# OpenGene/repaq

Hardware: AMD Instinct MI355X
Metric: raw FASTQ MB/s encode+decode (higher is better)
Workload: dtype u8; 1 GPU; configs[2]: synthetic NovaSeq PE150 two files (-i/-I), 2 x 4.01 GB FASTQ (fqgen profile 1, 11200000 pairs, seed 3, N 20 ppm), -k 1000, encode + decode; chunks_per_gpu=3360, parity=unchecked (checked with --full)

## Files before the change

### repaq_amd/csrc/enc/chunk_flags_overlap.h

```cpp
#pragma once
struct Layout {
    uint32_t off_readlens, off_n1lens, off_n2lens, off_stlens, off_lanes, off_tiles, off_x, off_y, off_n1, off_n2, off_st, off_seq, off_qual, off_ov, off_npos;
    uint32_t total, msize, seq_size, qual_size, npos_size, n1_size, n2_size, st_size, x_size, y_size, n_reads, flags;
};
__device__ __forceinline__ uint32_t name2_len_of(const Text& T, const ReadTab& R, uint32_t g) { return line_len(T, g, 0) - R.name2_off[g]; }

#define CF_ALL 0x3FFu
__global__ void k_chunk_flags_a(Text T, ReadTab R, ChunkTab C, const DevHeader* __restrict__ D, int is_pe, uint32_t* __restrict__ cbits, uint32_t* __restrict__ cfail) {
    __shared__ uint8_t s_names[4 * 65 * NAME_STRIDE];
    const uint32_t c = blockIdx.y, f = C.first[c], e = C.first[c + 1];
    const int l = lane_id(), w = wave_id(); const uint32_t wpb = blockDim.x >> 6;
    uint8_t* rows = s_names + (size_t)w * 65 * NAME_STRIDE;
    const bool can0 = is_pe && D->support_interleaved; const uint32_t dpos = D->name2_diff_pos, dch = D->name2_diff_char;
    const uint32_t nl0 = line_len(T, f, 0); const uint8_t* nm0g = line_ptr(T, f, 0);
    const uint32_t n1l0 = R.name1_len[f], n2o0 = R.name2_off[f], n2l0 = nl0 - n2o0, len0 = R.len[f], stl0 = line_len(T, f, 2);
    const uint8_t* st0 = line_ptr(T, f, 2); const uint8_t lane0 = R.lane[f]; const uint16_t tile0 = R.tile[f];
    { const uint32_t take = nl0 < NAME_CAP ? nl0 : NAME_CAP; for (uint32_t i = (uint32_t)l; i < take; i += 64) rows[64 * NAME_STRIDE + i] = nm0g[i]; }
    const uint8_t* nm0 = nl0 <= NAME_CAP ? rows + 64 * NAME_STRIDE : nm0g;
    uint32_t bits = CF_ALL, fail = 0xFFFFFFFFu;
    for (uint32_t gb = f + (blockIdx.x * wpb + (uint32_t)w) * 64u; gb < e; gb += gridDim.x * wpb * 64u) {
        const uint32_t g = gb + (uint32_t)l; const bool v = g < e;
        uint32_t nb = 0, nl = 0, stb = 0, stl = 0; int s = 0;
        if (v) { uint32_t r; read_loc(T, g, s, r); const uint32_t* p = t_lo(T, s) + 4 * (size_t)r; nb = p[0]; nl = p[1] - 1 - nb; stb = p[2]; stl = p[3] - 1 - stb; }
        wave_lds_sync();
// ... 81 lines not shown
}
#define OV2_CROW_OF(capb) ((capb) / 4u + 4u)
#define OV2_NROW_OF(capb) ((capb) == 256u ? 36u : (capb) / 8u + 8u)
#define OV2_FILTER 8
__device__ __forceinline__ uint32_t bfe_u32(uint32_t v, uint32_t off, uint32_t wid) { return (v >> off) & ((1u << wid) - 1u); }
static __device__ __noinline__ uint4 ld16_edge(const uint8_t* __restrict__ base, long long off, uint64_t n) {
    uint32_t w[4] = { 0, 0, 0, 0 };
    for (int b = 0; b < 16; b++) { const long long a = off + b; if (a >= 0 && (uint64_t)a < n) w[b >> 2] |= (uint32_t)base[a] << (8 * (b & 3)); }
    return make_uint4(w[0], w[1], w[2], w[3]);
}
__device__ __forceinline__ void ov2_pack_r1(uint32_t w, uint32_t& code, uint32_t& nbits, uint32_t& bad) {
    const uint32_t idx = (w >> 1) & 0x03030303u;
    const uint32_t ok = eq_bytes_full(__builtin_amdgcn_perm(0u, 0x47544341u, idx), w);
    code = ((__builtin_amdgcn_perm(0u, 0x00020301u, idx) & ok) * 0x01041040u) >> 24;
    nbits = 0; bad = 0;
    if (ok != 0xFFFFFFFFu) { const uint32_t isn = eq_bytes_full(w, 0x4E4E4E4Eu); nbits = ((isn & 0x01010101u) * 0x01020408u) >> 24; bad = ~ok & ~isn; }
}
__device__ __forceinline__ void ov2_pack_rc(uint32_t w, uint32_t& code, uint32_t& nbits) {
    const uint32_t u = w & 0xDFDFDFDFu, idx = (u >> 1) & 0x03030303u;
    const uint32_t ok = eq_bytes_full(__builtin_amdgcn_perm(0u, 0x47544341u, idx), u);
    code = ((__builtin_amdgcn_perm(0u, 0x03010002u, idx) & ok) * 0x01041040u) >> 24;
    nbits = ((~ok & 0x01010101u) * 0x01020408u) >> 24;
}
struct OvLoose { const uint32_t* pq; const uint32_t* lpk; const uint16_t* lnb; const uint8_t* rflag; };
template <bool LOOSE, uint32_t CAPB = 256u> __global__ void __launch_bounds__(256) k_overlap(Text T, OvLoose Z, int16_t* __restrict__ ovraw, uint32_t n_pairs) {
    constexpr uint32_t OV2_CAP = CAPB, OV2_CROW = OV2_CROW_OF(CAPB), OV2_NROW = OV2_NROW_OF(CAPB), OV2_WAVE_BYTES = 128u * (OV2_CROW + OV2_NROW); constexpr int OV2_ND = (int)(CAPB / 16u);
    static_assert((OV2_CROW / 4u) % 2u == 1u && (OV2_NROW / 4u) % 2u == 1u && OV2_WAVE_BYTES % 16u == 0u, "row geometry");
    __shared__ uint32_t s_rows[4 * (OV2_WAVE_BYTES / 4) + 4]; __shared__ uint32_t s_bad[4][2];
    const int l = lane_id(), w = wave_id();
    uint8_t* const c1 = (uint8_t*)(s_rows + (size_t)w * (OV2_WAVE_BYTES / 4)); uint8_t* const c2 = c1 + 64u * OV2_CROW;
    uint8_t* const n1 = c2 + 64u * OV2_CROW; uint8_t* const n2 = n1 + 64u * OV2_NROW;
    for (uint32_t p0 = (blockIdx.x * 4u + (uint32_t)w) * 64u; p0 < n_pairs; p0 += gridDim.x * 256u) {
        const uint32_t p = p0 + (uint32_t)l; int len1 = -1, len2 = 0; uint32_t q1 = 0, q2 = 0; int s1 = 0, s2 = 0; uint32_t ld1 = 0, ld2 = 0;
        if (p < n_pairs) {
            const uint32_t g = 2u * p;
            if (LOOSE) { const uint32_t a = Z.pq[g], b = Z.pq[g + 1], c_ = Z.pq[g + 2]; len1 = (int)(b - a); len2 = (int)(c_ - b); ld1 = (a >> 4) + g;
                    ld2 = (b >> 4) + g + 1u; }
            else { uint32_t r; read_loc(T, g, s1, r); const uint32_t* pa = t_lo(T, s1) + 4 * (size_t)r; q1 = pa[1]; len1 = (int)(pa[2] - 1u - q1);
                              read_loc(T, g + 1, s2, r); const uint32_t* pb = t_lo(T, s2) + 4 * (size_t)r; q2 = pb[1]; len2 = (int)(pb[2] - 1u - q2); }
        }
        const bool slow = len1 >= 0 && ((uint32_t)len1 > OV2_CAP || (uint32_t)len2 > OV2_CAP), fast = len1 >= 0 && !slow;
        const int mx = wave_max(fast ? (len1 > len2 ? len1 : len2) : 0);
        if (l < 2) s_bad[w][l] = 0;
        wave_lds_sync();
        { uint4* z = (uint4*)c1; for (uint32_t i = (uint32_t)l; i < OV2_WAVE_BYTES / 16u; i += 64u) z[i] = make_uint4(0, 0, 0, 0); }
        wave_lds_sync();
        if (LOOSE) {
            const uint32_t nd_ = ((uint32_t)mx + 15u) >> 4;
            uint32_t* const r1w = (uint32_t*)(c1 + (uint32_t)l * OV2_CROW); uint32_t* const r2w = (uint32_t*)(c2 + (uint32_t)l * OV2_CROW);
            uint16_t* const m1w = (uint16_t*)(n1 + (uint32_t)l * OV2_NROW); uint16_t* const m2w = (uint16_t*)(n2 + (uint32_t)l * OV2_NROW);
            for (uint32_t j0 = 0; j0 < nd_; j0 += 4u) {
                uint32_t va[4], vb[4]; uint16_t ma[4], mb[4];
#pragma unroll
                for (uint32_t u = 0; u < 4u; u++) {
                    const uint32_t j = j0 + u; const bool o1 = fast && j < nd_ && 16u * j < (uint32_t)len1, o2 = fast && j < nd_ && 16u * j < (uint32_t)len2;
                    va[u] = o1 ? Z.lpk[ld1 + j] : 0u; ma[u] = o1 ? Z.lnb[ld1 + j] : (uint16_t)0; vb[u] = o2 ? Z.lpk[ld2 + j] : 0u;
                            mb[u] = o2 ? Z.lnb[ld2 + j] : (uint16_t)0;
                }
#pragma unroll
                for (uint32_t u = 0; u < 4u; u++) { const uint32_t j = j0 + u; if (fast && j < nd_) { r1w[j] = va[u]; m1w[j] = ma[u]; r2w[j] = vb[u]; m2w[j] = mb[u]; } }
            }
        } else {
        const uint32_t G = ((uint32_t)mx + 31u + 31u) >> 5, ntasks = 128u * G, ginv = G ? (65536u + G - 1u) / G : 0u;
            const uint32_t meta1 = (uint32_t)(len1 < 0 ? 0 : (len1 > 0xFFFF ? 0xFFFF : len1)) | ((uint32_t)s1 << 16) | (fast ? 1u << 17 : 0u);
            const uint32_t meta2 = (uint32_t)(len2 < 0 ? 0 : (len2 > 0xFFFF ? 0xFFFF : len2)) | ((uint32_t)s2 << 16);
            for (uint32_t t0 = 0; t0 < ntasks; t0 += 256u) {
                uint32_t v[4][8]; uint32_t row[4]; int L[4], pos0[4]; bool on[4], edge[4]; const uint8_t* src[4]; uint32_t at[4], lim[4];
    #pragma unroll
                for (int u = 0; u < 4; u++) {
                    const uint32_t t = t0 + 64u * (uint32_t)u + (uint32_t)l; row[u] = t < ntasks ? (t * ginv) >> 16 : 0u; const uint32_t j = t - row[u] * G;
                    const int srcl = (int)(row[u] & 63u); const bool second = row[u] >= 64u;
                    const uint32_t ma = __shfl(meta1, srcl), mb = __shfl(meta2, srcl), o1 = __shfl(q1, srcl), o2 = __shfl(q2, srcl);
                    const uint32_t mm = second ? mb : ma; const bool f = (ma >> 17) & 1u;
                    L[u] = (int)(mm & 0xFFFFu); const uint32_t q = second ? o2 : o1, m = q & 31u;
                    at[u] = (q & ~31u) + 32u * j;
                    on[u] = t < ntasks && f && at[u] < q + (uint32_t)L[u];
                    const int z = (int)((mm >> 16) & 1u); src[u] = t_fq(T, z); lim[u] = t_n(T, z);
                    pos0[u] = second ? L[u] - 32 * (int)j + (int)m - 32 : 32 * (int)j - (int)m;
                    edge[u] = on[u] && (unsigned long long)at[u] + 32ull > (unsigned long long)lim[u];
                }
// ... 191 lines not shown
```

### repaq_amd/csrc/enc/gather_tiles.h

```cpp
#pragma once
#define G2_CAP 23552u
#define G2_SE_OK 1
#define G2_CNT 256u
__device__ __forceinline__ uint32_t ctl_flags4(uint32_t w) { return (w - 0x10101010u) & ~w & 0x80808080u; }
struct __attribute__((packed, aligned(1))) GU16g { uint32_t a, b, c, d; };
__device__ __forceinline__ void pack4_codes(uint32_t w, uint32_t& code, uint32_t& nb, uint32_t& bad) {
    const uint32_t idx = (w >> 1) & 0x03030303u;
    const uint32_t ok = eq_bytes_full(__builtin_amdgcn_perm(0u, 0x47544341u, idx), w);
    code = ((__builtin_amdgcn_perm(0u, 0x00020301u, idx) & ok) * 0x01041040u) >> 24;
    nb = 0; bad = 0;
    if (ok != 0xFFFFFFFFu) { const uint32_t isn = eq_bytes_full(w, 0x4E4E4E4Eu); nb = ((isn & 0x01010101u) * 0x01020408u) >> 24;
            bad = (((~ok & ~isn) & 0x01010101u) * 0x01020408u) >> 24; }
}
__device__ __forceinline__ void pack4_codes_rc(uint32_t w, uint32_t& code, uint32_t& nb) {
    const uint32_t u = w & 0xDFDFDFDFu, idx = (u >> 1) & 0x03030303u;
    const uint32_t ok = eq_bytes_full(__builtin_amdgcn_perm(0u, 0x47544341u, idx), u);
    code = ((__builtin_amdgcn_perm(0u, 0x03010002u, idx) & ok) * 0x01041040u) >> 24;
    nb = ((~ok & 0x01010101u) * 0x01020408u) >> 24;
}
__device__ __forceinline__ bool pack16_fast(const uint32_t (&w)[4], uint32_t& code) {
    uint32_t diff = 0; code = 0;
#pragma unroll
    for (int i = 0; i < 4; i++) {
        const uint32_t idx = (w[i] >> 1) & 0x03030303u;
// ... 84 lines not shown
        if (!m.rc) {
            lds_get16(s_text, m.ssrc + (tail ? m.len - 16u : 16u * gi), w);
            if (nv0 < 16u && !tail) blank(nv0, 16u);
            if (!pack16_fast(w, code)) {
                uint32_t bad = 0; code = 0;
#pragma unroll
                for (int i = 0; i < 4; i++) { uint32_t c4, n4, b4; pack4_codes(w[i], c4, n4, b4); code |= c4 << (8 * i); nbits |= n4 << (4 * i); bad |= b4 << (4 * i); }
                if (bad) rflag[m.gi] = 1;
                if (CHK && (m.gi & 1u)) { if (ctl_flags4(w[0]) | ctl_flags4(w[1]) | ctl_flags4(w[2]) | ctl_flags4(w[3])) *s_bad = 1u; }
            }
        } else {
            lds_get16(s_text, tail ? m.ssrc : m.ssrc + m.len - 16u * gi - 16u, w);
            if (nv0 < 16u && !tail) blank(0u, 16u - nv0);
            if (pack16_fast(w, code)) code = ~g2_rev2x16(code);
            else {
                if (CHK && (m.gi & 1u)) { if (ctl_flags4(w[0]) | ctl_flags4(w[1]) | ctl_flags4(w[2]) | ctl_flags4(w[3])) *s_bad = 1u; }
                const uint32_t x0 = bswap32(w[3]), x1 = bswap32(w[2]), x2 = bswap32(w[1]), x3 = bswap32(w[0]); w[0] = x0; w[1] = x1; w[2] = x2; w[3] = x3; code = 0;
#pragma unroll
                for (int i = 0; i < 4; i++) { uint32_t c4, n4; pack4_codes_rc(w[i], c4, n4); code |= c4 << (8 * i); nbits |= n4 << (4 * i); }
            }
        }
        code >>= 2u * tsh; nbits >>= tsh;
        if (nv0 < 16u) { code &= (1u << (2u * nv0)) - 1u; nbits &= (1u << nv0) - 1u; }
        lpk[m.ld + gi] = code; lnb[m.ld + gi] = (uint16_t)nbits;
        if (nbits) rn[m.gi] = 1;
    }
}
__device__ __forceinline__ void g2_compose(const uint8_t* s_text, const G2Read& m, uint32_t part, uint32_t P, uint8_t* qd, uint32_t* __restrict__ lpk,
        uint16_t* __restrict__ lnb, uint8_t* __restrict__ rflag, uint8_t* __restrict__ rn, QualCount& qc) {
    if (!m.on) return;
    {
        const uint32_t n = m.len; uint8_t* const o = qd + m.qpos; const bool rc = m.rc;
        if (n >= 16u) {
            const uint32_t ng = (n + 15u) >> 4;
            for (uint32_t gi = part; gi < ng; gi += P) {
                uint32_t p0 = 16u * gi, dup = 0; if (p0 + 16u > n) { dup = p0 + 16u - n; p0 = n - 16u; }
                uint32_t w[4]; lds_get16(s_text, rc ? m.qsrc + n - p0 - 16u : m.qsrc + p0, w);
                if (rc) { const uint32_t x0 = bswap32(w[3]), x1 = bswap32(w[2]), x2 = bswap32(w[1]), x3 = bswap32(w[0]); w[0] = x0; w[1] = x1; w[2] = x2; w[3] = x3; }
                { GU16g v; v.a = w[0]; v.b = w[1]; v.c = w[2]; v.d = w[3]; *(GU16g*)(o + p0) = v; }
                if (!dup) qc.group(m.qpos + p0, w[0], w[1], w[2], w[3]);
                else for (uint32_t k = dup; k < 16u; k++) qc(m.qpos + p0 + k, (uint8_t)(w[k >> 2] >> (8u * (k & 3u))));
            }
        } else for (uint32_t i = part; i < n; i += P) { const uint8_t q = s_text[rc ? m.qsrc + n - 1u - i : m.qsrc + i]; o[i] = q; qc(m.qpos + i, q); }
    }
    g2_bases(s_text, m, part, P, lpk, lnb, rflag, rn, nullptr);
}
#define G2_REFN 256u
#define G2_REFS 128u
// ... 360 lines not shown
            g2_flush_masks(pl, M.pw, nd, dense3, s_carry, gpl, M.pstride, gw0, nw, !last_tile && (qend & 31u) != 0u, cur == gs && gs > f && (qbeg & 31u) != 0u,
                    last_tile && ge < e && (qend & 31u) != 0u,
                           (size_t)c * MAX_STREAMS * n_seg, n_seg, segm, segc);
        } else qual_flush(sh, sh_last, nrep, nslot, qc.seg0, c, nn_s, segm, segc, n_seg);
        b0 = b1; b1 = b2; b2 = b3;
    }
    if (parse) {
        const uint32_t bits = wave_and(acc.bits), fail = wave_min(acc.fail);
        if ((tid & 63u) == 0) { if (bits != CF_ALL) atomicAnd(&cbits[c], bits); if (fail != 0xFFFFFFFFu) atomicMin(&cfail[c], fail); }
    }
    if (mirror) {
        __syncthreads();
        if (tid == 0 && s_mctl != mwant) atomicOr(M.mirror_err, (uint32_t)DE_MIRROR_FAIL);
    }
    if (LANES) { __syncthreads(); if (tid == 0 && s_mctl) atomicOr(M.mirror_err, (uint32_t)DE_MIRROR_FAIL); }
}
__device__ __forceinline__ uint32_t dense_mask_of(const DevHeader* __restrict__ D, uint32_t nd) { uint32_t m = 0;
        for (uint32_t d = 0; d < nd; d++) m |= 1u << D->dense[d]; return m; }
__device__ __forceinline__ void k_rare_zero_chunk(uint32_t* __restrict__ planes, uint64_t pstride, uint32_t dense_mask, const uint32_t* __restrict__ pq,
        const uint32_t* __restrict__ first, const uint64_t* __restrict__ qbase, uint32_t c) {
    const uint32_t nw = (pq[first[c + 1]] - pq[first[c]] + 31u) >> 5; const size_t w0 = (size_t)(qbase[c] >> 5);
    for (uint32_t v = 0; v < G2_PLANES; v++) if (!((dense_mask >> v) & 1u)) for (uint32_t i = threadIdx.x; i < nw; i += blockDim.x) planes[(size_t)v * pstride + w0 + i] = 0u;
}
__global__ void k_gather_redo_reset(const uint32_t* __restrict__ only, uint32_t* __restrict__ segm, int* __restrict__ segc, uint32_t n_seg,
                                    uint32_t* __restrict__ xplane, uint64_t pstride, const DevHeader* __restrict__ D, uint32_t nd, const uint32_t* __restrict__ pq, const uint32_t* __restrict__ first, const uint64_t* __restrict__ qbase) {
    const uint32_t c = blockIdx.x; if (!only[c]) return;
    const size_t k = (size_t)c * MAX_STREAMS * n_seg;
    for (uint32_t i = threadIdx.x; i < MAX_STREAMS * n_seg; i += blockDim.x) { segm[k + i] = 0u; segc[k + i] = -1; }
    if (xplane) { k_rare_zero_chunk(xplane, pstride, dense_mask_of(D, nd), pq, first, qbase, c);
            if (threadIdx.x == 0) xplane[(size_t)G2_PLANES * pstride + (size_t)c * (1u + G2_RARE_LIST)] = 0u; }
}
__global__ void k_rare_cleanup(uint32_t* __restrict__ rare, uint32_t* __restrict__ planes, uint64_t pstride, const DevHeader* __restrict__ D, uint32_t nd,
        const uint32_t* __restrict__ pq, const uint32_t* __restrict__ first, const uint64_t* __restrict__ qbase) {
    const uint32_t c = blockIdx.x; uint32_t* const rc = rare + (size_t)c * (1u + G2_RARE_LIST); const uint32_t n = rc[0]; if (!n) return;
    if (n <= G2_RARE_LIST) { const size_t w0 = (size_t)(qbase[c] >> 5); for (uint32_t i = threadIdx.x; i < n; i += blockDim.x) { const uint32_t e = rc[1u + i];
            planes[(size_t)(e >> 28) * pstride + w0 + (e & 0x0FFFFFFFu)] = 0u; } }
    else k_rare_zero_chunk(planes, pstride, dense_mask_of(D, nd), pq, first, qbase, c);
    __syncthreads();
    if (threadIdx.x == 0) rc[0] = 0u;
}
__device__ __forceinline__ uint32_t loose_codes(const uint32_t* __restrict__ lpk, uint32_t ld, uint32_t b) {
    const uint32_t d = ld + (b >> 4), sh = 2u * (b & 15u); const uint32_t lo = lpk[d];
    return sh ? (uint32_t)(((((unsigned long long)lpk[d + 1]) << 32) | lo) >> sh) : lo;
}
__device__ __forceinline__ uint32_t loose_nbits(const uint16_t* __restrict__ lnb, uint32_t ld, uint32_t b) {
    const uint32_t d = ld + (b >> 4), sh = b & 15u; const uint32_t lo = lnb[d];
    return (sh ? ((((uint32_t)lnb[d + 1]) << 16) | lo) >> sh : lo) & 0xFFFFu;
}
#define SP_OWN 4096u
#define SP_EXTRA 8u
#define SP_U 3
struct __attribute__((packed, aligned(4))) SpU8 { uint32_t a, b; };
struct __attribute__((packed, aligned(2))) SpU4 { uint32_t a; };
__global__ void __launch_bounds__(256) k_seqpack(const uint32_t* __restrict__ pq, const uint32_t* __restrict__ sd, const U4* __restrict__ ptot,
        const uint32_t* __restrict__ first, const uint32_t* __restrict__ ilv, const int8_t* __restrict__ ovb,
                                                 const DevHeader* __restrict__ D, const uint64_t* __restrict__ sbase, const uint32_t* __restrict__ lpk, const uint16_t* __restrict__ lnb, const uint8_t* __restrict__ rn,
                                                 uint32_t* __restrict__ spk, uint16_t* __restrict__ snm, uint32_t* __restrict__ ncount, uint32_t* __restrict__ nmap, uint32_t* __restrict__ segm, int* __restrict__ segc, uint32_t n_seg,
                                                 uint32_t rshift) {
    __shared__ uint32_t s_sd[256 + SP_EXTRA + 1], s_ld[256 + SP_EXTRA], s_sk[256 + SP_EXTRA]; __shared__ uint8_t s_own[SP_OWN];
    __shared__ uint8_t s_hn[256 + SP_EXTRA + 8];
    const uint32_t c = blockIdx.y, f = first[c], e = first[c + 1], tid = threadIdx.x;
    const uint32_t ps0 = sd[f], S = ptot[c].d;
// ... 139 lines not shown
```

### repaq_amd/csrc/rfq_ctx.h

```cpp
#pragma once
#include "rfq_common.h"
#include "../../include/rfq_hip.h"
#include <cstring>
#include <string>
#include <vector>
#include <cstdio>
#include <cstdarg>
#include <algorithm>

struct DBuf {
    void* p = nullptr; size_t cap = 0;
    hipError_t ensure(size_t n) {
        if (n <= cap) return hipSuccess;
        if (p) { (void)hipFree(p); p = nullptr; cap = 0; }
        size_t want = n + n / 4 + 4096;
        hipError_t e = hipMalloc(&p, want);
        if (e != hipSuccess) { p = nullptr; return e; }
        cap = want; return hipSuccess;
    }
    hipError_t ensure_keep(size_t n, size_t keep, hipStream_t s) {
        if (n <= cap) return hipSuccess;
        void* q = nullptr; const size_t want = n + n / 2 + 4096;
        hipError_t e = hipMalloc(&q, want);
        if (e != hipSuccess) return e;
// ... 95 lines not shown
        pend.push_back(Pend{ host, off, n }); pin_used = off + n;
        return hipMemcpyAsync(pin + off, dev, n, hipMemcpyDeviceToHost, s);
    }
    hipError_t fetch_sync(hipStream_t s) {
        const hipError_t e = hipStreamSynchronize(s);
        if (e == hipSuccess) for (const Pend& q : pend) memcpy(q.host, pin + q.off, q.n);
        pend.clear(); pin_used = 0;
        return e;
    }
    DBuf d_hdr;
    DevHeader h_hdr; bool have_hdr = false;
    bool hdr_on_device = false; uint8_t* pin_up = nullptr; hipEvent_t ev_up = nullptr; bool ev_up_pending = false;
    DBuf d_status; DevStatus h_status;
    DBuf d_cmp;
    DBuf b[120];
    DBuf out_img, out_fq1, out_fq2, out_acc, out_acc1, out_acc2;
    double rec_per_byte = 0.0; bool lazy_block = false;
    bool retried_room = false;
    bool mixed_lengths = false;
    bool dense_ok = false;
    void new_file() { dense_ok = false; e3_pieces_failed = false; mixed_lengths = false; mirror_block = false; }
    bool mirror_block = false, mirror_fell = false;
    bool qplane_dirty = true;
    uint32_t qplane_nd = 0, qplane_mask = 0;
    size_t qplane_stride = 0;
    DBuf rows_off[2], rows_stat, rows_txt[2];
    DBuf names_blob, names_off;
    std::vector<uint64_t> chunk_off;
    std::vector<uint64_t> scan_end[2];
    StageTimer timer;
};

static inline int rfq_fail(rfq_ctx* c, int code, const char* fmt, ...) {
    char buf[1024]; va_list ap; va_start(ap, fmt); vsnprintf(buf, sizeof buf, fmt, ap); va_end(ap);
    if (c) c->err = buf;
    return code;
}
#define HIPCHK(ctx, call) do { hipError_t e_ = (call); if (e_ != hipSuccess) return rfq_fail(ctx, RFQ_E_HIP, "%s failed: %s", #call, hipGetErrorString(e_)); } while (0)
#define KCHK(ctx, what) do { hipError_t e_ = hipGetLastError(); if (e_ != hipSuccess) return rfq_fail(ctx, RFQ_E_HIP, "launch of %s failed: %s", what, hipGetErrorString(e_)); } while (0)

static inline uint32_t rows_vec(uint64_t row_len, const void* p, const void* q) { return (row_len % 16u == 0 && !(((uintptr_t)p | (uintptr_t)q) & 15u)) ? 1u : 0u; }

#define SCAN_TPB 256
#define SCAN_ITEMS 8
#define SCAN_TILE (SCAN_TPB * SCAN_ITEMS)

// ... 66 lines not shown
```

### repaq_amd/csrc/rfq_encode.hip

```cpp
#include "rfq_ctx.h"
#include <type_traits>
#include "rfq_encode_kernels.h"
#include <algorithm>
#include <cstring>
#include <cstdlib>
#include <cstddef>

enum EncBuf {
    B_BITMAP0 = 0, B_BITMAP1, B_BLK0, B_BLK1, B_LO0, B_LO1, B_SCANTMP,
    B_LEN, B_N1LEN, B_N2OFF, B_X, B_Y, B_TILE, B_LANE, B_OK, B_CHUNK, B_STORED, B_EQ2, B_PQ, B_PV, B_PVIN,
    B_ULEN, B_P, B_MINMAX, B_FIRST, B_CFLAGS, B_IL, B_HIST, B_NCOUNT, B_SCAP, B_SOFF, B_SSIZE, B_XSIZE, B_YSIZE, B_QBASE, B_SBASE,
    B_IMGSIZE, B_IMGOFF, B_CTOTAL, B_CBASE, B_LAYOUT, B_HSTATS, B_OVB, B_OVRAW, B_QCAT, B_SCAT, B_SCRATCH, B_XS, B_YS, B_SEGB, B_SEGC,
    B_NORM0, B_NORM1, B_OT0, B_OT1, B_ONX0, B_ONX1, B_TBITS, B_SBITS, B_NKEEP, B_NTERM, B_NMAP, B_ADJ, B_PINFO, B_SEGM, B_LPK, B_LNB, B_SPK, B_SNM, B_RFLAG, B_SCANTMP2, B_CTOTALN, B_CBASEN, B_SCRATCHN, B_PTOT, B_QPLANE, B_SEGD, B_SEGS, B_SD, B_RN, B_ENC_END
};

static_assert(B_ENC_END <= 80, "encode buffers must stay below the decode buffer indices of rfq_ctx::b");

static int fetch_bytes(rfq_ctx* ctx, const uint8_t* d, size_t n, std::string& out) {
    out.resize(n);
    if (n) HIPCHK(ctx, hipMemcpy(&out[0], d, n, hipMemcpyDeviceToHost));
    return RFQ_OK;
}
static int fetch_line(rfq_ctx* ctx, const Text& T, uint32_t g, int k, std::string& out) {
    int s = 0; uint32_t r = g; if (T.paired == 1) { s = (int)(g & 1u); r = g >> 1; }
// ... 365 lines not shown
}
static void chunk_layout(hipStream_t Q, const EncBatch& b, const EncCut& cut, const EncTables& t, uint64_t* tmp, int exact) {
    hipLaunchKernelGGL(k_chunk_layout, dim3((cut.n_chunks + 63) / 64), dim3(64), 0, Q, b.T, t.R, t.C, (const DevHeader*)t.D, t.L, cut.n_chunks, exact, b.dst);
    scan_exclusive<uint64_t>(Q, t.C.img_size, t.C.img_off, cut.n_chunks, tmp, 1);
}
static int enc_gather_tiles(rfq_ctx* ctx, const EncBatch& b, const EncCut& cut, EncTables& t, EncForm& f, AuxGuard& guard) {
    hipStream_t S = ctx->stream; DBuf* B = ctx->b;
    const uint32_t np = cut.reads_used / 2;
    if (b.mirrored && f.masks && !G2_SE_OK) return RFQ_AGAIN_MIRROR;
    uint8_t *rflag, *rn; HIPCHK(ctx, table(B[B_RFLAG], (t.nr + 15) & ~(size_t)15, rflag)); HIPCHK(ctx, table(B[B_RN], (t.nr + 15) & ~(size_t)15, rn));
    ClearList z; memset(&z, 0, sizeof z);
    if (!(z.add(t.cbits, 2 * t.nc * 4, 0xFFFFFFFFu) && z.add(t.C.ncount, t.nc * 4, 0u) && z.add(t.C.nmap, t.nc * NMAP_WORDS * 4, 0u) && z.add(t.segb, t.nsb * 4, 0u) &&
          z.add(t.segm, t.nsb * 4, 0u) && z.add(t.segc, t.nsb * 4, 0xFFFFFFFFu) && z.add(rflag, t.nr, 0u) && z.add(rn, t.nr, 0u)))
        return rfq_fail(ctx, RFQ_E_HIP, "internal: more than %d regions in one clear list", CLEAR_MAX);
    clear_list(S, z);
    ctx->timer.begin("chunk_flags", S);
    hipLaunchKernelGGL(k_chunk_bases, dim3((cut.n_chunks + 255) / 256), dim3(256), 0, S, t.R, t.C, cut.n_chunks, 1);
    if (f.hdr_aside) HIPCHK(ctx, hipStreamWaitEvent(S, ctx->ev_mid, 0));
    ctx->timer.end(S);

    if (f.masks) { ctx->timer.begin("quality_masks", S); ctx->timer.end(S); }
    ctx->timer.begin("gather", S);
    const size_t nld = (size_t)(cut.total_bases >> 4) + cut.reads_used + 16;
    uint32_t* lpk; uint16_t* lnb; HIPCHK(ctx, table(B[B_LPK], nld * 4, lpk)); HIPCHK(ctx, table(B[B_LNB], nld * 2, lnb));
    const uint32_t K = 1u << f.kshift;
    const uint32_t bx = grid_x_for(cut.n_chunks, (cut.max_reads + K - 1) / K, 6u * ctx->n_cu);
    const uint32_t text4 = (uint32_t)((((uint64_t)cut.max_rec << f.kshift) + 64u + 15u) / 16u) + 8u;
    G2Planes M; M.planes = nullptr; M.rare = nullptr; M.pstride = 0; M.nd = 0; M.mirror_err = b.mirrored ? &b.dst->err : (uint32_t*)nullptr; M.pw = (uint32_t)((((uint64_t)cut.max_len << f.kshift) + 31u) / 32u) + 2u;
    auto dyn_of = [&](uint32_t nd_) -> uint32_t { return text4 * 16u + (G2_REFN + G2_REFS + 32u) + 4u * nd_ * M.pw; };
    if (f.masks) {
        M.nd = std::min<uint32_t>(ctx->h_hdr.n_normal, 3u);
        if (M.nd == 3u && dyn_of(3u) + 64u > 26880u) M.nd = 2u;
        const size_t need_w = (t.catbytes >> 5) + 16, extra_w = t.nc * (1u + G2_RARE_LIST) / G2_PLANES + 16;
        if (B[B_QPLANE].cap / 4 / G2_PLANES < need_w + extra_w || ctx->qplane_stride < need_w) {
            HIPCHK(ctx, B[B_QPLANE].ensure((need_w + extra_w) * G2_PLANES * 4)); ctx->qplane_stride = B[B_QPLANE].cap / 4 / G2_PLANES - extra_w;
                    ctx->qplane_dirty = true;
        }
        if ((ctx->qplane_stride + extra_w) * G2_PLANES * 4 > B[B_QPLANE].cap) { ctx->qplane_stride = B[B_QPLANE].cap / 4 / G2_PLANES - extra_w;
                ctx->qplane_dirty = true; }
        uint32_t dmask = 0; for (uint32_t d = 0; d < M.nd; d++) dmask |= 1u << (ctx->h_hdr.dense[d] & 7u);
        if (ctx->qplane_mask & ~dmask) ctx->qplane_dirty = true;
        ctx->qplane_mask = dmask;
        M.planes = B[B_QPLANE].as<uint32_t>(); M.pstride = ctx->qplane_stride; M.rare = M.planes + G2_PLANES * M.pstride;
        if (ctx->qplane_dirty) HIPCHK(ctx, hipMemsetAsync(M.planes, 0, ((size_t)M.pstride * G2_PLANES + t.nc * (1u + G2_RARE_LIST)) * 4, S));
        ctx->qplane_dirty = true; ctx->qplane_nd = M.nd;
    }
    t.qplane = f.masks ? M.planes : nullptr;
    const uint32_t dyn = dyn_of(M.nd) + ctx->opt.g2_pad; (void)dyn;
    for (int phase = 1; phase <= (b.is_pe ? 2 : 1); phase++) {
        const uint32_t* only = phase == 2 ? (const uint32_t*)t.redo : (const uint32_t*)nullptr;
        if (phase == 2) hipLaunchKernelGGL(k_gather_redo_reset, dim3(cut.n_chunks), dim3(64), 0, S, only, t.segm, t.segc, t.n_seg,
                                           f.masks ? M.planes : (uint32_t*)nullptr, M.pstride, (const DevHeader*)t.D, M.nd, (const uint32_t*)t.R.pq, (const uint32_t*)t.C.first, (const uint64_t*)t.C.qbase);
        if (f.masks) hipLaunchKernelGGL(k_mask_bounds, dim3(cut.n_chunks), dim3(64), 0, S, (const uint32_t*)t.R.pq, (const uint32_t*)t.C.first, (const uint64_t*)t.C.qbase,
                M.planes, M.pstride, (const DevHeader*)t.D, M.nd, bx, only);
#define RFQ_G2_ARGS b.T, t.R, (const uint32_t*)t.C.first, (const uint64_t*)t.C.qbase, (const DevHeader*)t.D, t.qcat, lpk, lnb, rflag, \
                    rn, t.segm, t.segc, t.n_seg, f.kshift, t.cbits, t.cfail, only, text4, M
        if (f.masks && !b.is_pe && G2_SE_OK) hipLaunchKernelGGL((k_gather2<true, 0>), dim3(bx, cut.n_chunks), dim3(256), dyn, S, RFQ_G2_ARGS);
        else if (f.masks && b.a->paired == RFQ_PE_TWO_FILES && G2_SE_OK && b.mirrored) hipLaunchKernelGGL((k_gather2<true, 1, true>), dim3(bx, cut.n_chunks), dim3(256), dyn, S, RFQ_G2_ARGS);
        else if (f.masks && b.a->paired == RFQ_PE_TWO_FILES && G2_SE_OK) hipLaunchKernelGGL((k_gather2<true, 1>), dim3(bx, cut.n_chunks), dim3(256), dyn, S, RFQ_G2_ARGS);
        else if (f.masks) hipLaunchKernelGGL(k_gather2<true>, dim3(bx, cut.n_chunks), dim3(256), dyn, S, RFQ_G2_ARGS);
        else hipLaunchKernelGGL(k_gather2<false>, dim3(bx, cut.n_chunks), dim3(256), dyn, S, RFQ_G2_ARGS);
#undef RFQ_G2_ARGS
        if (phase == 1) hipLaunchKernelGGL(k_chunk_flags_b, dim3(cut.n_chunks), dim3(64), 0, S, t.R, t.C, (const DevHeader*)t.D, b.is_pe ? 1 : 0, (const uint32_t*)t.cbits,
                (const uint32_t*)t.cfail, t.redo);
    }
    HIPCHK(ctx, table(B[B_SCRATCH], std::max<size_t>(B[B_SCRATCH].cap, (size_t)(f.masks ? cut.total_bases / 8 : cut.total_bases + cut.total_bases / 4) + t.nc * 4096 + 256), t.scratch));
    HIPCHK(ctx, table(B[B_SCRATCHN], std::max<size_t>(B[B_SCRATCHN].cap, (size_t)(cut.total_bases / 64) + t.nc * 1024 + 256), t.scratch_n));
    hipLaunchKernelGGL(k_stream_plan, dim3(cut.n_chunks), dim3(64), 0, S, t.R, t.C, (const DevHeader*)t.D, t.ctot, t.ctot_n, cut.n_chunks, (const uint32_t*)t.segm, t.n_seg, 1);
    scan_exclusive<uint64_t>(S, t.ctot, t.cbase, cut.n_chunks, (uint64_t*)t.scantmp, 1);
    hipLaunchKernelGGL(k_enc_totals, dim3(1), dim3(64), 0, S, t.C, (const uint64_t*)t.cbase, cut.n_chunks, 0, b.dst, (uint64_t)B[B_SCRATCH].cap);
    const bool aux_chain = f.aux_chain = ctx->aux_ready() && !ctx->opt.one_stream; hipStream_t A = aux_chain ? ctx->aux : S;
    if (aux_chain) { HIPCHK(ctx, hipEventRecord(ctx->ev_fork, S)); HIPCHK(ctx, hipStreamWaitEvent(A, ctx->ev_fork, 0)); guard.armed = true; }
    if (b.is_pe) {
        const OvLoose Z = { (const uint32_t*)t.R.pq, (const uint32_t*)lpk, (const uint16_t*)lnb, (const uint8_t*)rflag };
        const uint32_t ob = std::min<uint32_t>((np + 255) / 256, 65535u * 16u);
        if (cut.max_len <= 160u) hipLaunchKernelGGL((k_overlap<true, 160u>), dim3(ob), dim3(256), 0, A, b.T, Z, t.ovraw, np);
        else hipLaunchKernelGGL(k_overlap<true>, dim3(ob), dim3(256), 0, A, b.T, Z, t.ovraw, np);
    }
    if (aux_chain) { HIPCHK(ctx, hipEventRecord(ctx->ev_ovl, A)); f.coder_waits = true; }
    hipLaunchKernelGGL(k_chunk_prefix, dim3(cut.n_chunks), dim3(256), 0, A, b.T, t.R, t.C, (const DevHeader*)t.D, (const int16_t*)t.ovraw, t.ovb);
    {
        const uint32_t max_len = cut.max_rec / 2u;
        uint32_t rshift = 8; while (rshift && ((uint64_t)(max_len / 16u + 1u) << rshift) > SP_OWN) rshift--;
        uint32_t sx = grid_x_for(cut.n_chunks, (cut.max_reads >> rshift) + 1u, 8u * ctx->n_cu);
        hipLaunchKernelGGL(k_seqpack, dim3(sx, cut.n_chunks), dim3(256), aux_chain ? ctx->opt.sp_pad : 0u, A, (const uint32_t*)t.R.pq, (const uint32_t*)t.R.sd, (const U4*)t.C.ptot,
                (const uint32_t*)t.C.first, (const uint32_t*)t.C.il, (const int8_t*)t.ovb, (const DevHeader*)t.D,
                           (const uint64_t*)t.C.sbase, (const uint32_t*)lpk, (const uint16_t*)lnb, (const uint8_t*)rn, t.spk, t.snm,
                           t.C.ncount, t.C.nmap, t.segm, t.segc, t.n_seg, rshift);
    }
    uint64_t* tmp2 = B[B_SCANTMP2].as<uint64_t>() + (t.nr / SCAN_TILE + 2) * 2;
    hipLaunchKernelGGL(k_stream_plan, dim3(cut.n_chunks), dim3(64), 0, A, t.R, t.C, (const DevHeader*)t.D, t.ctot, t.ctot_n, cut.n_chunks, (const uint32_t*)t.segm, t.n_seg, 2);
    scan_exclusive<uint64_t>(A, t.ctot_n, t.cbase_n, cut.n_chunks, tmp2, 1);
    chunk_layout(A, b, cut, t, tmp2, 0);
    hipLaunchKernelGGL(k_enc_totals, dim3(1), dim3(64), 0, A, t.C, (const uint64_t*)t.cbase_n, cut.n_chunks, 2, b.dst, (uint64_t)B[B_SCRATCHN].cap);
    KCHK(ctx, "k_gather2");
    ctx->timer.end(S);
    return RFQ_OK;
}
static int enc_gather_bytes(rfq_ctx* ctx, EncBatch& b, const EncCut& cut, EncTables& t, EncForm& f) {
    hipStream_t S = ctx->stream; DBuf* B = ctx->b;
    uint64_t* const tmp = (uint64_t*)t.scantmp;
    HIPCHK(ctx, hipMemsetAsync(t.cbits, 0xFF, 2 * t.nc * 4, S));
    ctx->timer.begin("chunk_flags", S);
    hipLaunchKernelGGL(k_chunk_bases, dim3((cut.n_chunks + 255) / 256), dim3(256), 0, S, t.R, t.C, cut.n_chunks, 1);
    if (f.hdr_aside) HIPCHK(ctx, hipStreamWaitEvent(S, ctx->ev_mid, 0));
    const uint32_t fbx = std::max(1u, std::min<uint32_t>((cut.max_reads + 255) / 256, std::max(1u, 4096u / cut.n_chunks)));
    hipLaunchKernelGGL(k_chunk_flags_a, dim3(fbx, cut.n_chunks), dim3(256), 0, S, b.T, t.R, t.C, (const DevHeader*)t.D, b.is_pe ? 1 : 0, t.cbits, t.cfail);
    hipLaunchKernelGGL(k_chunk_flags_b, dim3(cut.n_chunks), dim3(64), 0, S, t.R, t.C, (const DevHeader*)t.D, b.is_pe ? 1 : 0, (const uint32_t*)t.cbits, (const uint32_t*)t.cfail,
            (uint32_t*)nullptr);
    if (b.is_pe) {
        const OvLoose noz = { nullptr, nullptr, nullptr, nullptr };
        const uint32_t ob = std::min<uint32_t>((cut.n_units + 255) / 256, 65535u * 16u);
        hipLaunchKernelGGL(k_overlap<false>, dim3(ob), dim3(256), 0, S, b.T, noz, t.ovraw, cut.n_units);
    }
    const uint32_t np = cut.reads_used / 2; U4* const pvin = B[B_PVIN].as<U4>();
    if (b.is_pe) hipLaunchKernelGGL(k_overlap_apply, dim3((np + 255) / 256), dim3(256), 0, S, t.R, t.C, (const DevHeader*)t.D, (const int16_t*)t.ovraw, t.ovb, np);
    hipLaunchKernelGGL(k_pv_in, dim3((cut.n_reads + 255) / 256), dim3(256), 0, S, b.T, t.R, pvin, cut.n_reads);
    scan_exclusive<U4>(S, pvin, t.R.pv, cut.n_reads, (U4*)t.scantmp, 1);
    hipLaunchKernelGGL(k_chunk_bases, dim3((cut.n_chunks + 255) / 256), dim3(256), 0, S, t.R, t.C, cut.n_chunks, 2);
    hipLaunchKernelGGL(k_chunk_ptot, dim3((cut.n_chunks + 255) / 256), dim3(256), 0, S, t.R, t.C, cut.n_chunks);
    KCHK(ctx, "k_chunk_flags");
    ctx->timer.end(S);

    ctx->timer.begin("gather_bytes", S);
    HIPCHK(ctx, hipMemsetAsync(t.C.ncount, 0, t.nc * 4, S)); HIPCHK(ctx, hipMemsetAsync(t.C.nmap, 0, t.nc * NMAP_WORDS * 4, S));
    HIPCHK(ctx, hipMemsetAsync(t.segb, 0, t.nsb * 4, S)); HIPCHK(ctx, hipMemsetAsync(t.segm, 0, t.nsb * 4, S));
            HIPCHK(ctx, hipMemsetAsync(t.segc, 0xFF, t.nsb * 4, S));
    uint8_t* scat; HIPCHK(ctx, table(B[B_SCAT], t.catbytes, scat));
    const uint32_t bx = grid_x_for(cut.n_chunks, (cut.max_reads + GT_READS - 1) / GT_READS, 5u * ctx->n_cu);
    hipLaunchKernelGGL(k_gather, dim3(bx, cut.n_chunks), dim3(256), 0, S, b.T, t.R, t.C, (const int8_t*)t.ovb, (const DevHeader*)t.D, t.qcat, scat, t.segm, t.segc, t.n_seg);
    const uint32_t px = grid_x_for(cut.n_chunks, (cut.max_chunk_bases / 16u + 255u) / 256u + 1u, 8u * ctx->n_cu);
    hipLaunchKernelGGL(k_packbytes, dim3(px, cut.n_chunks), dim3(256), 0, S, (const U4*)t.R.pv, (const uint32_t*)t.C.first, (const uint64_t*)t.C.sbase, (const uint8_t*)scat,
                       t.spk, t.snm);
    hipLaunchKernelGGL(k_stream_plan, dim3(cut.n_chunks), dim3(64), 0, S, t.R, t.C, (const DevHeader*)t.D, t.ctot, t.ctot_n, cut.n_chunks, (const uint32_t*)t.segm, t.n_seg, 3);
// ... 38 lines not shown
        if (f.coder_waits) HIPCHK(ctx, hipStreamWaitEvent(S, ctx->ev_ovl, 0));
        { const int rc = launch_coder(ctx, S, b, cut, t, f, 0, f.nqg + 1); if (rc) return rc; }
        hipLaunchKernelGGL(k_coords, dim3(2, cut.n_chunks), dim3(64), 0, S, t.R, t.C, (const DevHeader*)t.D, t.xs, t.ys, b.dst);
    } else if (fork_coords) { HIPCHK(ctx, hipEventRecord(ctx->ev_fork, S)); HIPCHK(ctx, hipStreamWaitEvent(ctx->aux, ctx->ev_fork, 0)); }
    t.hdr_bytes = b.a->emit_header ? ctx->h_hdr.len : 0;
    if (b.a->d_out) { t.img = b.a->d_out; t.img_cap = b.a->out_cap; } else {
        const size_t nb_all = b.nbytes[0] + b.nbytes[1];
        const size_t want = f.fast ? std::max<size_t>(ctx->out_img.cap, (f.masks ? nb_all / 3 : nb_all - nb_all / 8) + (1u << 20)) : (size_t)(b.hs.image_bound + t.hdr_bytes + 64);
        HIPCHK(ctx, ctx->out_img.ensure(want)); t.img = ctx->out_img.as<uint8_t>(); t.img_cap = ctx->out_img.cap;
    }
    if (t.hdr_bytes) {
        if (t.img_cap < t.hdr_bytes) return rfq_fail(ctx, RFQ_E_NOSPACE, "output buffer too small for the header");
        HIPCHK(ctx, hipMemcpyAsync(t.img, ctx->h_hdr.bytes, t.hdr_bytes, hipMemcpyHostToDevice, S));
    }
    hipStream_t A2 = (f.fast ? f.aux_chain : fork_coords) ? ctx->aux : S;
    if (f.fast) { const int rc = launch_coder(ctx, A2, b, cut, t, f, f.nqg + 1, 1); if (rc) return rc; }
    else { hipLaunchKernelGGL(k_coords, dim3(2, cut.n_chunks), dim3(64), 0, A2, t.R, t.C, (const DevHeader*)t.D, t.xs, t.ys, b.dst); const int rc = launch_coder(ctx, S, b, cut, t, f, 0, f.nqg + 2); if (rc) return rc; }
    if (A2 != S) { HIPCHK(ctx, hipEventRecord(ctx->ev_join, A2)); HIPCHK(ctx, hipStreamWaitEvent(S, ctx->ev_join, 0)); }
    KCHK(ctx, "k_pos_coder");
    if (f.masks) {
        hipLaunchKernelGGL(k_rare_cleanup, dim3(cut.n_chunks), dim3(256), 0, S, t.qplane + G2_PLANES * ctx->qplane_stride, t.qplane, (uint64_t)ctx->qplane_stride,
                           (const DevHeader*)t.D, ctx->qplane_nd, (const uint32_t*)t.R.pq, (const uint32_t*)t.C.first, (const uint64_t*)t.C.qbase);
        ctx->qplane_dirty = false;
    }
    ctx->timer.end(S);
    return RFQ_OK;
}
static int enc_assemble(rfq_ctx* ctx, const EncBatch& b, const EncCut& cut, EncTables& t) {
    hipStream_t S = ctx->stream; DBuf* B = ctx->b;
    ctx->timer.begin("coords+layout", S);
    uint32_t *segd, *segs; HIPCHK(ctx, table(B[B_SEGD], t.nsb * 4, segd)); HIPCHK(ctx, table(B[B_SEGS], t.nsb * 4, segs));
    hipLaunchKernelGGL(k_pos_sizes, dim3(cut.n_chunks), dim3(64), 0, S, t.C, (const DevHeader*)t.D, (const uint32_t*)t.segb, (const uint32_t*)t.segm, t.n_seg, segd, segs);
    chunk_layout(S, b, cut, t, (uint64_t*)t.scantmp, 1);
    hipLaunchKernelGGL(k_enc_totals, dim3(1), dim3(64), 0, S, t.C, (const uint64_t*)t.cbase, cut.n_chunks, 1, b.dst, ~0ull);
    KCHK(ctx, "k_coords");
    ctx->timer.end(S);
    ctx->timer.begin("assemble", S);
    const uint32_t tail_bases = ((b.a->final && !b.a->flush_all) || b.ended) ? b.a->chunk_bases : 0u;
    const uint32_t bpc = grid_x_for(cut.n_chunks, 64u, 8u * ctx->n_cu);
    hipLaunchKernelGGL(k_assemble, dim3(bpc, cut.n_chunks), dim3(256), 0, S, b.T, t.R, t.C, (const DevHeader*)t.D, (const Layout*)t.L,
                       (const uint8_t*)t.qcat, (const uint32_t*)t.spk, (const uint8_t*)t.scratch, (const uint64_t*)t.cbase,
                       (const uint8_t*)t.scratch_n, (const uint64_t*)t.cbase_n,
                       (const uint8_t*)t.xs, (const uint8_t*)t.ys, (const int8_t*)t.ovb, t.img, t.img_cap, t.hdr_bytes,
                       b.a->file_off1, b.a->file_off2, b.a->nolb_from1, b.a->nolb_from2,
                       (const uint32_t*)t.segb, (const uint32_t*)segd, (const uint32_t*)segs, t.n_seg, b.dst,
                       tail_bases, cut.units_used, cut.nlines[0], cut.nlines[1], b.orig_n(0), b.orig_n(1));
// ... 795 lines not shown
```

Before: 1.177 million MB/s.

## Write N-bit masks only for reads with Ns, keep lnb buffer zero across batches

The gather kernel now stores the per-word N-bit mask only when a word actually holds an N. The mask buffer is instead kept all-zero across batches: it is fully memset on first use or after a realloc, and a cleanup kernel re-zeroes only the slots of reads flagged in rn. The overlap kernel also reads the mask only for reads whose rn flag is set. This removes most 16-bit mask writes and reads for low-N data. In exchange it adds a dirty-state invariant across batches, a cleanup kernel and a reset in the redo phase, and any path that skips the cleanup could leave stale masks behind.

Result: faster. 1.199 million MB/s (median of 6 runs) (+1.9%).

```diff
diff --git a/repaq_amd/csrc/enc/chunk_flags_overlap.h b/repaq_amd/csrc/enc/chunk_flags_overlap.h
--- a/repaq_amd/csrc/enc/chunk_flags_overlap.h
+++ b/repaq_amd/csrc/enc/chunk_flags_overlap.h
@@ -127,7 +127,7 @@
     code = ((__builtin_amdgcn_perm(0u, 0x03010002u, idx) & ok) * 0x01041040u) >> 24;
     nbits = ((~ok & 0x01010101u) * 0x01020408u) >> 24;
 }
-struct OvLoose { const uint32_t* pq; const uint32_t* lpk; const uint16_t* lnb; const uint8_t* rflag; };
+struct OvLoose { const uint32_t* pq; const uint32_t* lpk; const uint16_t* lnb; const uint8_t* rflag; const uint8_t* rn; };
 template <bool LOOSE, uint32_t CAPB = 256u> __global__ void __launch_bounds__(256) k_overlap(Text T, OvLoose Z, int16_t* __restrict__ ovraw, uint32_t n_pairs) {
     constexpr uint32_t OV2_CAP = CAPB, OV2_CROW = OV2_CROW_OF(CAPB), OV2_NROW = OV2_NROW_OF(CAPB), OV2_WAVE_BYTES = 128u * (OV2_CROW + OV2_NROW); constexpr int OV2_ND = (int)(CAPB / 16u);
     static_assert((OV2_CROW / 4u) % 2u == 1u && (OV2_NROW / 4u) % 2u == 1u && OV2_WAVE_BYTES % 16u == 0u, "row geometry");
@@ -144,6 +144,8 @@
             else { uint32_t r; read_loc(T, g, s1, r); const uint32_t* pa = t_lo(T, s1) + 4 * (size_t)r; q1 = pa[1]; len1 = (int)(pa[2] - 1u - q1);
                               read_loc(T, g + 1, s2, r); const uint32_t* pb = t_lo(T, s2) + 4 * (size_t)r; q2 = pb[1]; len2 = (int)(pb[2] - 1u - q2); }
         }
+        bool h1 = false, h2 = false;
+        if (LOOSE && p < n_pairs) { const uint32_t hh = *(const uint16_t*)(Z.rn + 2u * (size_t)p); h1 = (hh & 0xFFu) != 0u; h2 = (hh >> 8) != 0u; }
         const bool slow = len1 >= 0 && ((uint32_t)len1 > OV2_CAP || (uint32_t)len2 > OV2_CAP), fast = len1 >= 0 && !slow;
         const int mx = wave_max(fast ? (len1 > len2 ? len1 : len2) : 0);
         if (l < 2) s_bad[w][l] = 0;
@@ -159,8 +161,8 @@
 #pragma unroll
                 for (uint32_t u = 0; u < 4u; u++) {
                     const uint32_t j = j0 + u; const bool o1 = fast && j < nd_ && 16u * j < (uint32_t)len1, o2 = fast && j < nd_ && 16u * j < (uint32_t)len2;
-                    va[u] = o1 ? Z.lpk[ld1 + j] : 0u; ma[u] = o1 ? Z.lnb[ld1 + j] : (uint16_t)0; vb[u] = o2 ? Z.lpk[ld2 + j] : 0u;
-                            mb[u] = o2 ? Z.lnb[ld2 + j] : (uint16_t)0;
+                    va[u] = o1 ? Z.lpk[ld1 + j] : 0u; ma[u] = o1 && h1 ? Z.lnb[ld1 + j] : (uint16_t)0; vb[u] = o2 ? Z.lpk[ld2 + j] : 0u;
+                            mb[u] = o2 && h2 ? Z.lnb[ld2 + j] : (uint16_t)0;
                 }
 #pragma unroll
                 for (uint32_t u = 0; u < 4u; u++) { const uint32_t j = j0 + u; if (fast && j < nd_) { r1w[j] = va[u]; m1w[j] = ma[u]; r2w[j] = vb[u]; m2w[j] = mb[u]; } }
diff --git a/repaq_amd/csrc/enc/gather_tiles.h b/repaq_amd/csrc/enc/gather_tiles.h
--- a/repaq_amd/csrc/enc/gather_tiles.h
+++ b/repaq_amd/csrc/enc/gather_tiles.h
@@ -130,8 +130,8 @@
         }
         code >>= 2u * tsh; nbits >>= tsh;
         if (nv0 < 16u) { code &= (1u << (2u * nv0)) - 1u; nbits &= (1u << nv0) - 1u; }
-        lpk[m.ld + gi] = code; lnb[m.ld + gi] = (uint16_t)nbits;
-        if (nbits) rn[m.gi] = 1;
+        lpk[m.ld + gi] = code;
+        if (nbits) { lnb[m.ld + gi] = (uint16_t)nbits; rn[m.gi] = 1; }
     }
 }
 __device__ __forceinline__ void g2_compose(const uint8_t* s_text, const G2Read& m, uint32_t part, uint32_t P, uint8_t* qd, uint32_t* __restrict__ lpk,
@@ -538,9 +538,15 @@
     const uint32_t nw = (pq[first[c + 1]] - pq[first[c]] + 31u) >> 5; const size_t w0 = (size_t)(qbase[c] >> 5);
     for (uint32_t v = 0; v < G2_PLANES; v++) if (!((dense_mask >> v) & 1u)) for (uint32_t i = threadIdx.x; i < nw; i += blockDim.x) planes[(size_t)v * pstride + w0 + i] = 0u;
 }
+__device__ __forceinline__ void nbits_zero_slots(uint16_t* __restrict__ lnb, const uint8_t* __restrict__ rn, const uint32_t* __restrict__ pq, uint32_t g0, uint32_t g1, uint32_t t, uint32_t n) {
+    for (uint32_t g = g0 + t; g < g1; g += n) if (rn[g]) { const uint32_t a = pq[g], nw = (pq[g + 1] - a + 15u) >> 4; uint16_t* const o = lnb + (size_t)(a >> 4) + g;
+            for (uint32_t i = 0; i < nw; i++) o[i] = 0; }
+}
 __global__ void k_gather_redo_reset(const uint32_t* __restrict__ only, uint32_t* __restrict__ segm, int* __restrict__ segc, uint32_t n_seg,
-                                    uint32_t* __restrict__ xplane, uint64_t pstride, const DevHeader* __restrict__ D, uint32_t nd, const uint32_t* __restrict__ pq, const uint32_t* __restrict__ first, const uint64_t* __restrict__ qbase) {
+                                    uint32_t* __restrict__ xplane, uint64_t pstride, const DevHeader* __restrict__ D, uint32_t nd, const uint32_t* __restrict__ pq, const uint32_t* __restrict__ first, const uint64_t* __restrict__ qbase,
+                                    uint16_t* __restrict__ lnb, const uint8_t* __restrict__ rn) {
     const uint32_t c = blockIdx.x; if (!only[c]) return;
+    nbits_zero_slots(lnb, rn, pq, first[c], first[c + 1], threadIdx.x, blockDim.x);
     const size_t k = (size_t)c * MAX_STREAMS * n_seg;
     for (uint32_t i = threadIdx.x; i < MAX_STREAMS * n_seg; i += blockDim.x) { segm[k + i] = 0u; segc[k + i] = -1; }
     if (xplane) { k_rare_zero_chunk(xplane, pstride, dense_mask_of(D, nd), pq, first, qbase, c);
@@ -554,6 +560,12 @@
     else k_rare_zero_chunk(planes, pstride, dense_mask_of(D, nd), pq, first, qbase, c);
     __syncthreads();
     if (threadIdx.x == 0) rc[0] = 0u;
+}
+__global__ void __launch_bounds__(256) k_nbits_cleanup(uint16_t* __restrict__ lnb, const uint8_t* __restrict__ rn, const uint32_t* __restrict__ pq, uint32_t n_reads) {
+    const uint32_t g0 = 16u * (blockIdx.x * blockDim.x + threadIdx.x); if (g0 >= n_reads) return;
+    const uint4 v = *(const uint4*)(rn + g0);
+    if (!(v.x | v.y | v.z | v.w)) return;
+    nbits_zero_slots(lnb, rn, pq, g0, g0 + 16u < n_reads ? g0 + 16u : n_reads, 0u, 1u);
 }
 __device__ __forceinline__ uint32_t loose_codes(const uint32_t* __restrict__ lpk, uint32_t ld, uint32_t b) {
     const uint32_t d = ld + (b >> 4), sh = 2u * (b & 15u); const uint32_t lo = lpk[d];
diff --git a/repaq_amd/csrc/rfq_ctx.h b/repaq_amd/csrc/rfq_ctx.h
--- a/repaq_amd/csrc/rfq_ctx.h
+++ b/repaq_amd/csrc/rfq_ctx.h
@@ -141,6 +141,7 @@
     void new_file() { dense_ok = false; e3_pieces_failed = false; mixed_lengths = false; mirror_block = false; }
     bool mirror_block = false, mirror_fell = false;
     bool qplane_dirty = true;
+    bool lnb_dirty = true;
     uint32_t qplane_nd = 0, qplane_mask = 0;
     size_t qplane_stride = 0;
     DBuf rows_off[2], rows_stat, rows_txt[2];
diff --git a/repaq_amd/csrc/rfq_encode.hip b/repaq_amd/csrc/rfq_encode.hip
--- a/repaq_amd/csrc/rfq_encode.hip
+++ b/repaq_amd/csrc/rfq_encode.hip
@@ -411,7 +411,11 @@
     if (f.masks) { ctx->timer.begin("quality_masks", S); ctx->timer.end(S); }
     ctx->timer.begin("gather", S);
     const size_t nld = (size_t)(cut.total_bases >> 4) + cut.reads_used + 16;
+    const size_t lnb_cap = B[B_LNB].cap;
     uint32_t* lpk; uint16_t* lnb; HIPCHK(ctx, table(B[B_LPK], nld * 4, lpk)); HIPCHK(ctx, table(B[B_LNB], nld * 2, lnb));
+    if (B[B_LNB].cap != lnb_cap) ctx->lnb_dirty = true;
+    if (ctx->lnb_dirty) HIPCHK(ctx, hipMemsetAsync(lnb, 0, B[B_LNB].cap, S));
+    ctx->lnb_dirty = true;
     const uint32_t K = 1u << f.kshift;
     const uint32_t bx = grid_x_for(cut.n_chunks, (cut.max_reads + K - 1) / K, 6u * ctx->n_cu);
     const uint32_t text4 = (uint32_t)((((uint64_t)cut.max_rec << f.kshift) + 64u + 15u) / 16u) + 8u;
@@ -439,7 +443,8 @@
     for (int phase = 1; phase <= (b.is_pe ? 2 : 1); phase++) {
         const uint32_t* only = phase == 2 ? (const uint32_t*)t.redo : (const uint32_t*)nullptr;
         if (phase == 2) hipLaunchKernelGGL(k_gather_redo_reset, dim3(cut.n_chunks), dim3(64), 0, S, only, t.segm, t.segc, t.n_seg,
-                                           f.masks ? M.planes : (uint32_t*)nullptr, M.pstride, (const DevHeader*)t.D, M.nd, (const uint32_t*)t.R.pq, (const uint32_t*)t.C.first, (const uint64_t*)t.C.qbase);
+                                           f.masks ? M.planes : (uint32_t*)nullptr, M.pstride, (const DevHeader*)t.D, M.nd, (const uint32_t*)t.R.pq, (const uint32_t*)t.C.first, (const uint64_t*)t.C.qbase,
+                                           lnb, (const uint8_t*)rn);
         if (f.masks) hipLaunchKernelGGL(k_mask_bounds, dim3(cut.n_chunks), dim3(64), 0, S, (const uint32_t*)t.R.pq, (const uint32_t*)t.C.first, (const uint64_t*)t.C.qbase,
                 M.planes, M.pstride, (const DevHeader*)t.D, M.nd, bx, only);
 #define RFQ_G2_ARGS b.T, t.R, (const uint32_t*)t.C.first, (const uint64_t*)t.C.qbase, (const DevHeader*)t.D, t.qcat, lpk, lnb, rflag, \
@@ -461,7 +466,7 @@
     const bool aux_chain = f.aux_chain = ctx->aux_ready() && !ctx->opt.one_stream; hipStream_t A = aux_chain ? ctx->aux : S;
     if (aux_chain) { HIPCHK(ctx, hipEventRecord(ctx->ev_fork, S)); HIPCHK(ctx, hipStreamWaitEvent(A, ctx->ev_fork, 0)); guard.armed = true; }
     if (b.is_pe) {
-        const OvLoose Z = { (const uint32_t*)t.R.pq, (const uint32_t*)lpk, (const uint16_t*)lnb, (const uint8_t*)rflag };
+        const OvLoose Z = { (const uint32_t*)t.R.pq, (const uint32_t*)lpk, (const uint16_t*)lnb, (const uint8_t*)rflag, (const uint8_t*)rn };
         const uint32_t ob = std::min<uint32_t>((np + 255) / 256, 65535u * 16u);
         if (cut.max_len <= 160u) hipLaunchKernelGGL((k_overlap<true, 160u>), dim3(ob), dim3(256), 0, A, b.T, Z, t.ovraw, np);
         else hipLaunchKernelGGL(k_overlap<true>, dim3(ob), dim3(256), 0, A, b.T, Z, t.ovraw, np);
@@ -498,7 +503,7 @@
     hipLaunchKernelGGL(k_chunk_flags_b, dim3(cut.n_chunks), dim3(64), 0, S, t.R, t.C, (const DevHeader*)t.D, b.is_pe ? 1 : 0, (const uint32_t*)t.cbits, (const uint32_t*)t.cfail,
             (uint32_t*)nullptr);
     if (b.is_pe) {
-        const OvLoose noz = { nullptr, nullptr, nullptr, nullptr };
+        const OvLoose noz = { nullptr, nullptr, nullptr, nullptr, nullptr };
         const uint32_t ob = std::min<uint32_t>((cut.n_units + 255) / 256, 65535u * 16u);
         hipLaunchKernelGGL(k_overlap<false>, dim3(ob), dim3(256), 0, S, b.T, noz, t.ovraw, cut.n_units);
     }
@@ -583,6 +588,12 @@
         hipLaunchKernelGGL(k_rare_cleanup, dim3(cut.n_chunks), dim3(256), 0, S, t.qplane + G2_PLANES * ctx->qplane_stride, t.qplane, (uint64_t)ctx->qplane_stride,
                            (const DevHeader*)t.D, ctx->qplane_nd, (const uint32_t*)t.R.pq, (const uint32_t*)t.C.first, (const uint64_t*)t.C.qbase);
         ctx->qplane_dirty = false;
+    }
+    if (f.fast) {
+        hipLaunchKernelGGL(k_nbits_cleanup, dim3((cut.reads_used + 4095u) / 4096u), dim3(256), 0, S, B[B_LNB].as<uint16_t>(), (const uint8_t*)B[B_RN].as<uint8_t>(),
+                           (const uint32_t*)t.R.pq, cut.reads_used);
+        KCHK(ctx, "k_nbits_cleanup");
+        ctx->lnb_dirty = false;
     }
     ctx->timer.end(S);
     return RFQ_OK;
```
